# grossmanlev/FL-distributed-delay

Measured on AMD Instinct MI355X. Metric: simulated worker-steps/sec (node) @1024 workers, delay 50; aggregation HBM GB/s, higher is better.
Workload: dtype f32

## Files before the change

### fl-distributed-delay_amd/csrc/common.h

```cpp
#pragma once
#include <hip/hip_runtime.h>
#include <stdint.h>
#include <stdlib.h>

#define FLSIM_WAVE 64

#if !defined(FLSIM_LAB) &&                                                                  \
    (defined(FLSIM_X6_FRESH) || defined(FLSIM_X6_PP_V) || defined(FLSIM_DG_FMS) ||          \
     defined(FLSIM_DIRECT_FENCES) || defined(FLSIM_DX6_FENCES) || defined(FLSIM_BUFLOAD) ||  \
     defined(FLSIM_SEQ_EARLY_EXIT) || defined(FLSIM_X6_FLUSH) || defined(FLSIM_WGRAD_X6) ||     \
     defined(FLSIM_ZL1F) || defined(FLSIM_SINGLE_BUF) || defined(FLSIM_DG3_FM) || defined(FLSIM_DX_FM))
#error "FLSIM_* measurement overrides need a lab build (make LAB=1)"
#endif

typedef float f32x4 __attribute__((ext_vector_type(4)));

namespace flsim {

void set_error(const char* fmt, ...);
const char* last_error();

#define FLSIM_CHECK_HIP(expr)                                                           \
    do {                                                                                \
        hipError_t _e = (expr);                                                         \
        if (_e != hipSuccess) {                                                         \
            ::flsim::set_error("%s failed: %s (%s:%d)", #expr, hipGetErrorString(_e),   \
                               __FILE__, __LINE__);                                     \
            return 2;                                                                   \
        }                                                                               \
    } while (0)

#define FLSIM_REQUIRE(cond, ...)                                                        \
    do {                                                                                \
        if (!(cond)) {                                                                  \
            ::flsim::set_error(__VA_ARGS__);                                            \
            return 1;                                                                   \
        }                                                                               \
    } while (0)

#define RC(x) do { int _r = (x); if (_r) return _r; } while (0)

inline const char* lab_env(const char* name) {
#ifdef FLSIM_LAB
    return getenv(name);
// ... 54 lines not shown
```

### fl-distributed-delay_amd/csrc/gemm_direct.h

```cpp
#pragma once
#include "loaders.h"

namespace flsim {

#ifndef FLSIM_DIRECT_FENCES
#define FLSIM_DIRECT_FENCES 1
#endif
constexpr bool DIRECT_FENCES = FLSIM_DIRECT_FENCES;

template <int IH, int IW, int CI, int PAD, int FM, bool WIN = false, int OHX = 0,
          class SRC = BufSrc>
struct Im2colDirect {
    using Unit = typename SRC::Unit;
    static constexpr int PIX = SRC::SM ? GK : CI;
    static constexpr int SLICE = SRC::SM ? IH * IW * GK : GK;
    static constexpr int OH = OHX > 0 ? OHX : IH + 2 * PAD - 2;
    static constexpr int OW = OHX > 0 ? OHX : IW + 2 * PAD - 2;
    static constexpr int PH = OH / 2, PW = OW / 2;
    static constexpr int ROWS_PER_IMG = WIN ? 4 * PH * PW : OH * OW;
    static_assert(CI % 16 == 0, "direct A needs whole 16-channel slices");

    const float* X;
    const float* XL = nullptr;
    int M;
    unsigned vb[FM];
    unsigned short tapmask[FM];
    SRC buf;

    __device__ void setup(int r0, int lane) {
        const int q = lane >> 4;
        buf.init(X, XL, (unsigned long)((M + ROWS_PER_IMG - 1) / ROWS_PER_IMG) * IH * IW * CI * 4);
#pragma unroll
        for (int f = 0; f < FM; ++f) {
            const int m = r0 + 16 * f + (lane & 15);
            long base = 0;
            int msk = 0;
            if (m < M) {
                const int nimg = m / ROWS_PER_IMG;
                const int rem = m - nimg * ROWS_PER_IMG;
                int oh, ow;
                if constexpr (WIN) {
                    const int qq = rem >> 2;
                    const int ph = qq / PW;
                    oh = 2 * ph + ((rem >> 1) & 1);
                    ow = 2 * (qq - ph * PW) + (rem & 1);
                } else {
                    oh = rem / OW;
                    ow = rem - oh * OW;
                }
                base = (long)nimg * IH * IW * CI + ((long)(oh - PAD) * IW + (ow - PAD)) * PIX +
                       4 * q;
#pragma unroll
                for (int t = 0; t < 9; ++t) {
                    const int ih = oh + t / 3 - PAD, iw = ow + t % 3 - PAD;
                    if ((unsigned)ih < (unsigned)IH && (unsigned)iw < (unsigned)IW) msk |= 1 << t;
                }
            }
            vb[f] = (unsigned)base * 4u;
            tapmask[f] = (unsigned short)msk;
        }
    }
    __device__ void load(int ks, Unit (&r)[FM]) const {
        const int cs = ks / 9;
        const int khkw = ks - 9 * cs;
        const int kh = khkw / 3;
        const unsigned off = (unsigned)(((kh * IW + (khkw - 3 * kh)) * PIX + cs * SLICE) * 4);
#pragma unroll
        for (int f = 0; f < FM; ++f) r[f] = buf.ld_or0(vb[f] + off, (tapmask[f] >> khkw) & 1);
    }
};

template <int TR, int NT>
struct RowsKCStage {
    static constexpr int ROWS = TR;
    static constexpr bool KC = true;
    static constexpr int TOTAL = ROWS * 4;
    static constexpr int UNITS = (TOTAL + NT - 1) / NT;
    static constexpr int FLOATS = KCTile<ROWS>::FLOATS + 4;
    const float* P;
    long ld;
    int NR;
    unsigned rowb[UNITS];
    int dst[UNITS];
    BufSrc buf;
    __device__ void setup(int r0, int tid) {
        buf.init(P, (unsigned long)NR * ld * 4);
#pragma unroll
        for (int j = 0; j < UNITS; ++j) {
            const int u0 = tid + j * NT;
            const bool real = u0 < TOTAL;
            const int u = real ? u0 : u0 % TOTAL;
            const int r = u >> 2, q = u & 3;
            rowb[j] = r0 + r < NR ? (unsigned)(((long)(r0 + r) * ld + 4 * q) * 4) : BUF_OOB;
            dst[j] = real ? KCTile<ROWS>::chunk_off(r, q) : KCTile<ROWS>::FLOATS;
        }
    }
    __device__ void load(int ks, f32x4 (&r)[UNITS]) const {
#pragma unroll
        for (int j = 0; j < UNITS; ++j)
            r[j] = buf.ld(rowb[j] == BUF_OOB ? BUF_OOB : rowb[j] + (unsigned)(ks * GK * 4));
    }
    __device__ void store(float* lds, const f32x4 (&r)[UNITS]) const {
// ... 125 lines not shown
```

### fl-distributed-delay_amd/csrc/gemm_dx6.h

```cpp
#pragma once
#include "gemm_direct.h"
#include "gemm_x6.h"

namespace flsim {

#ifndef FLSIM_DX6_FENCES
#define FLSIM_DX6_FENCES 1
#endif
constexpr bool DX6_FENCES = FLSIM_DX6_FENCES;

template <int TR, int NT, int NPL>
struct RowsKCStageXs {
    using Unit = XsUnit;
    static constexpr int ROWS = TR;
    static constexpr bool KC = true;
    static constexpr int TOTAL = ROWS * 4;
    static constexpr int UNITS = (TOTAL + NT - 1) / NT;
    static constexpr int PLANE = KCTile<ROWS>::FLOATS;
    static constexpr int SPARE = NPL * PLANE;
    static constexpr int FLOATS = NPL * PLANE + 4;
    static_assert(NPL == 2 || NPL == 3, "");
    const float* P;
    const float* PL;
    long ld;
// ... 44 lines not shown
    constexpr int STAGE_LD = BN + 4;
    constexpr int BASE_FL = 2 * STG;
    constexpr int WROWS = 16 * FM;
    constexpr int WM_FIT = (BASE_FL > 8192 ? BASE_FL : 8192) / (WROWS * STAGE_LD);
    constexpr int WM_PASS = WM_FIT < 1 ? 1 : (WM_FIT > WAVES ? WAVES : WM_FIT);
    constexpr int LDS_FL = STAGED && WM_PASS * WROWS * STAGE_LD > BASE_FL
                               ? WM_PASS * WROWS * STAGE_LD : BASE_FL;
    static_assert(LDS_FL * 4 <= 160 * 1024, "LDS");
    __shared__ __attribute__((aligned(16))) float lds[LDS_FL];

    const int tid = threadIdx.x;
    const int lane = tid & 63;
    const int wave = tid >> 6;
    const int nb = gridDim.x;
    const int b = blockIdx.x;
    const int q = nb / 8, r = nb % 8, xcd = b % 8;
    const int L = (xcd < r ? xcd * (q + 1) : r * (q + 1) + (xcd - r) * q) + b / 8;
    const int tn = L % tiles_n;
    const int tm = L / tiles_n;
    const int m0 = tm * BM;
    const int n0 = tn * BN;

    ad.setup(m0 + wave * WROWS, lane);
    bl.setup(n0, tid);

    f32x4 acc[FM][FN];
#pragma unroll
    for (int i = 0; i < FM; ++i)
#pragma unroll
        for (int j = 0; j < FN; ++j) acc[i][j] = f32x4{0.f, 0.f, 0.f, 0.f};

    constexpr int R = DEPTH + 1;
    static_assert(KB % R == 0, "the A register ring index must be static");
    XsUnit ra[R][FM];
    typename BL::Unit rb[BL::UNITS];
    const int nst = ksteps / KB;
#pragma unroll
    for (int d = 0; d < DEPTH; ++d) ad.load(d, ra[d]);
#pragma unroll
    for (int kk = 0; kk < KB; ++kk) {
        bl.load(kk, rb);
        bl.store(lds + kk * BFL, rb);
    }
    __syncthreads();
    if constexpr (WAVES == 8) {
        if (wave >= 4) __builtin_amdgcn_s_setprio(1);
    }
    for (int s = 0; s < nst; ++s) {
        const float* Bs = lds + (s & 1) * STG;
        float* Bn = lds + ((s + 1) & 1) * STG;
        const int kn = (s + 1) * KB;
#pragma unroll
        for (int kk = 0; kk < KB; ++kk) {
            const int ks = s * KB + kk;
            if (kk > 0) bl.store(Bn + (kk - 1) * BFL, rb);
            bl.load(kn + kk, rb);
            ad.load(ks + DEPTH, ra[(kk + DEPTH) % R]);
            if constexpr (DX6_FENCES) __builtin_amdgcn_sched_barrier(0);
            const float* Bk = Bs + kk * BFL;
            f32x4 a0[FM], a1[FM];
#pragma unroll
            for (int i = 0; i < FM; ++i) {
                a0[i] = ra[kk % R][i].hm;
                a1[i] = xs_hl(ra[kk % R][i]);
            }
#pragma unroll
            for (int j = 0; j < FN; ++j) {
                const f32x4 x0 = read_frag<true, BN>(Bk, 16 * j, lane);
                const f32x4 x2 = read_frag<true, BN>(Bk + PLANE, 16 * j, lane);
                f32x4 x1;
                if constexpr (BFL >= 3 * PLANE)
                    x1 = read_frag<true, BN>(Bk + 2 * PLANE, 16 * j, lane);
                else
                    x1 = f32x4{x0.z, x0.w, x0.x, x0.y};
#pragma unroll
                for (int i = 0; i < FM; ++i) {
                    acc[i][j] = x6_step<x6_fresh(true)>(acc[i][j], a0[i], a1[i], x0, x1, x2);
                }
            }
            if constexpr (DX6_FENCES) __builtin_amdgcn_sched_barrier(0);
        }
        bl.store(Bn + (KB - 1) * BFL, rb);
        __syncthreads();
    }

    if constexpr (STAGED) {
        static_assert(BN == EPI::NCOL || (IsPartial<EPI>::value && EPI::NCOL % BN == 0),
                      "staged epilogue needs the full row in one block");
        constexpr int PASSES = (WAVES + WM_PASS - 1) / WM_PASS;
#pragma unroll 1
        for (int pass = 0; pass < PASSES; ++pass) {
            __syncthreads();
            if (wave / WM_PASS == pass) {
#pragma unroll
                for (int i = 0; i < FM; ++i)
#pragma unroll
                    for (int j = 0; j < FN; ++j) {
                        const int ml = (wave - pass * WM_PASS) * WROWS + 16 * i + 4 * (lane >> 4);
                        const int nl = 16 * j + (lane & 15);
#pragma unroll
                        for (int rr = 0; rr < 4; ++rr)
                            lds[(ml + rr) * STAGE_LD + nl] = epi.value(nl, acc[i][j][rr]);
                    }
            }
            __syncthreads();
            const int w_hi = (pass + 1) * WM_PASS < WAVES ? (pass + 1) * WM_PASS : WAVES;
            staged_store(epi, lds, STAGE_LD, m0 + pass * WM_PASS * WROWS,
                         (w_hi - pass * WM_PASS) * WROWS, n0, BN, tid, 64 * WAVES);
        }
    } else {
#pragma unroll
        for (int i = 0; i < FM; ++i)
#pragma unroll
            for (int j = 0; j < FN; ++j) {
                const int m = m0 + wave * WROWS + 16 * i + 4 * (lane >> 4);
                const int n = n0 + 16 * j + (lane & 15);
// ... 7 lines not shown
```

### fl-distributed-delay_amd/csrc/net_kernels.h

```cpp
#pragma once
#include "epi_xs.h"
#include "gemm_direct.h"
#include "gemm_dx6.h"
#include "gemm_x6.h"
#include "loaders.h"
#include "pn1.h"
#include "probe.h"

namespace flsim {

static __global__ void __launch_bounds__(256)
k_fill_batch(const uint8_t* __restrict__ pool, const int32_t* __restrict__ labels,
             const int32_t* __restrict__ list_a, int len_a, const int32_t* __restrict__ list_b,
             int len_b, const WorkerRec* __restrict__ workers, int n_workers_total, uint64_t seed,
             const float* __restrict__ lut, float* __restrict__ x0, int32_t* __restrict__ y) {
    const int s = blockIdx.x;
    const int w = s / SAMPLES_PER_WORKER;
    const int j = s - w * SAMPLES_PER_WORKER;
    const WorkerRec wr = workers[w];
    const uint32_t bsz = wr.pad ? wr.pad : (uint32_t)SAMPLES_PER_WORKER;
    const uint32_t q = (wr.i >> 20) * SAMPLES_PER_WORKER + (uint32_t)j;
    float* out = x0 + (long)s * 4096;
    if (q >= bsz) {
        if (threadIdx.x == 0) y[s] = -1;
// ... 810 lines not shown
    al.NC = CO;
    BL bl;
    bl.X = X;
    bl.M = M;
    EpiSlabAccRing epi{{slab, CO, KP, (long)CO * KP, bslab, zinit}};
    const int tm = ceil_div(CO, BM), tn = KP / BN;
    static const int cap =
        resident_blocks((const void*)gemm_kernel<FM, FN, WM, WN, AL, BL, EpiSlabAccRing>, NT);
    const int ksteps = ceil_div(M, GK);
    const int zu = wsplit(ksteps, Z, tm * tn, cap);
    if (zused) *zused = zu;
    const int per = (ksteps + zu - 1) / zu;
    const ProbeSlot ps = probe_begin();
    hipExtLaunchKernelGGL((gemm_kernel<FM, FN, WM, WN, AL, BL, EpiSlabAccRing>), dim3(tm * tn * zu),
                          dim3(NT), 0, st, ps.start, ps.stop, 0, al, bl, epi, ksteps, per, tm, tn);
    FLSIM_LAUNCH_CHECK();
    return probe_end(ps, kid, 2.0 * M * CO * kreal);
}

template <int IH, int IW, int CI, int PAD, int FM, int FN, int WM, int WN, int FMS, int FNS,
          int WMS, int WNS, int VO = 0, bool DZC = false, bool X6 = false, class SRC = BufSrc,
          class SRCB = SRC>
static int conv_wgrad_sz(const float* dz, const float* X, int S, int CO, int KP, float* slab,
                         float* bslab, int Z, hipStream_t st, int kid, int kreal, int zinit,
                         int* zused, const float* dzl = nullptr, const float* Xl = nullptr) {
    if (S <= small_chunk_samples())
        return conv_wgrad<IH, IW, CI, PAD, FMS, FNS, WMS, WNS, VO, DZC, X6, SRC, SRCB>(
            dz, X, S, CO, KP, slab, bslab, Z, st, kid, kreal, zinit, zused, dzl, Xl);
    return conv_wgrad<IH, IW, CI, PAD, FM, FN, WM, WN, VO, DZC, X6, SRC, SRCB>(
        dz, X, S, CO, KP, slab, bslab, Z, st, kid, kreal, zinit, zused, dzl, Xl);
}

template <int IH, int IW, int CI, int PAD, int FM, int FN, int WAVES, int KB, int DEPTH, int NPL,
          bool WIN, int OHX, class ASRC = XsSrc, class EPI>
static int conv_dx6(XsT X, int S, XsT W, int N, int KP, const EPI& epi, hipStream_t st, int kid,
                    int kreal) {
    static_assert(ASRC::SPLIT, "split input");
    using AD = Im2colDirect<IH, IW, CI, PAD, FM, WIN, OHX, ASRC>;
    using BL = RowsKCStageXs<16 * FN, 64 * WAVES, NPL>;
    constexpr int BM = 16 * FM * WAVES, BN = 16 * FN;
    FLSIM_REQUIRE((KP / GK) % KB == 0, "direct GEMM: %d k-steps not a multiple of %d", KP / GK, KB);
    AD ad;
    ad.X = X.hm;
    ad.XL = X.l;
    ad.M = S * AD::ROWS_PER_IMG;
    BL bl;
    bl.P = W.hm;
    bl.PL = W.l;
    bl.ld = KP;
    bl.NR = N;
    const int tm = ceil_div(ad.M, BM), tn = ceil_div(N, BN);
    const ProbeSlot ps = probe_begin();
    hipExtLaunchKernelGGL((gemm_dx6_kernel<FM, FN, WAVES, KB, DEPTH, AD, BL, EPI>),
                          dim3(tm * tn), dim3(64 * WAVES), 0, st, ps.start, ps.stop, 0, ad, bl,
                          epi, KP / GK, tm, tn);
    FLSIM_LAUNCH_CHECK();
    return probe_end(ps, kid, 2.0 * ad.M * N * kreal);
}

template <int IH, int IW, int CI, int PAD, int FM, int FN, int WM, int WN, bool WIN, int OHX,
          class EPI>
static int conv_xs(XsT X, int S, XsT W, int N, int KP, const EPI& epi, hipStream_t st, int kid,
                   int kreal) {
    constexpr int NT = 64 * WM * WN;
    constexpr int BM = 16 * FM * WM, BN = 16 * FN * WN;
    using AL = Im2colKC<IH, IW, CI, PAD, BM, NT, WIN, OHX, XsSrc>;
    using BL = RowsKC<BN, NT, XsSrc>;
    AL al;
    al.X = X.hm;
    al.XL = X.l;
    al.M = S * AL::ROWS_PER_IMG;
// ... 77 lines not shown
```

### fl-distributed-delay_amd/csrc/pn1_net.hip

```cpp
#include <stdarg.h>
#include <stdio.h>
#include <string.h>

#include <mutex>
#include <unordered_map>

#include "net_kernels.h"
#include "slabstep.h"

namespace flsim {

static thread_local char g_err[512];
void set_error(const char* fmt, ...) {
    va_list ap;
    va_start(ap, fmt);
    vsnprintf(g_err, sizeof(g_err), fmt, ap);
    va_end(ap);
}
const char* last_error() { return g_err; }

struct ConvGeo {
    int CI, CIP, CO, H;
    int KP;
    int ZW;
// ... 214 lines not shown
#pragma unroll
                for (int r = 0; r < 4; ++r)
                    st[(16 * t + 4 * g + r) * C1_LD + 16 * j + i] = fmaxf(acc[t][j][r] + bj[j], 0.f);
        __builtin_amdgcn_wave_barrier();
#pragma unroll
        for (int q0 = 0; q0 < C1_ROWS * 12; q0 += 64) {
            const int q = q0 + lane, slice = q >> 7, row = (q & 127) >> 2, c4 = 4 * slice + (q & 3);
            xs_store_f(a1, a1l, a1f, xs_unit<48, 1156, true>((unsigned)(u * C1_ROWS + row), c4),
                       *reinterpret_cast<const f32x4*>(st + row * C1_LD + 4 * c4));
        }
        __builtin_amdgcn_wave_barrier();
    }
}

static int conv1_fwd(const float* x0, const float* W, const float* bias, XsT a1, float* a1f,
                     int S, hipStream_t st) {
    const long M = (long)S * 34 * 34;
    if (M % C1_ROWS) return 1;
    const long units = M / C1_ROWS;
    const int grid = (int)(units / 4 < 2048 ? (units + 3) / 4 : 2048);
    const ProbeSlot ps = probe_begin();
    hipExtLaunchKernelGGL(k_conv1_fwd, dim3(grid), dim3(256), 0, st, ps.start, ps.stop, 0, x0, W,
                          bias, a1.hm, a1.l, a1f, units);
    FLSIM_LAUNCH_CHECK();
    return probe_end(ps, K_FWD1, 2.0 * M * 48 * 27);
}

#ifndef FLSIM_DX_FM
#define FLSIM_DX_FM 4
#endif
constexpr int DX_FM = FLSIM_DX_FM, DX_FMS = 1, DX_KB = 3, DX_DEPTH = 2, DX_NPL = 2;


template <int IH, int IW, int CI, int PAD, int FN, bool WIN, int OHX, int FM = DX_FM,
          int WAVES = 8, int FMS = (FM == DX_FM ? DX_FMS : FM / 2), class EPI>
static int dx6(XsT X, int S, XsT W, int N, int KP, const EPI& epi, hipStream_t st, int kid,
               int kreal) {
    if (S <= small_chunk_samples())
        return conv_dx6<IH, IW, CI, PAD, FMS, FN, WAVES, DX_KB, DX_DEPTH, DX_NPL, WIN, OHX,
                        XsSrcSM>(X, S, W, N, KP, epi, st, kid, kreal);
    return conv_dx6<IH, IW, CI, PAD, FM, FN, WAVES, DX_KB, DX_DEPTH, DX_NPL, WIN, OHX, XsSrcSM>(
        X, S, W, N, KP, epi, st, kid, kreal);
}

template <int IH, int IW, int CI, int PAD, int FM, int FN, int WM, int WN, bool WIN, int OHX,
          class EPI>
static int xs(XsT X, int S, XsT W, int N, int KP, const EPI& epi, hipStream_t st, int kid,
              int kreal) {
    if (S <= small_chunk_samples())
        return conv_xs<IH, IW, CI, PAD, FM / 2, FN, WM, WN, WIN, OHX>(X, S, W, N, KP, epi, st, kid,
                                                                     kreal);
    return conv_xs<IH, IW, CI, PAD, FM, FN, WM, WN, WIN, OHX>(X, S, W, N, KP, epi, st, kid, kreal);
}

static int forward(const GradState& g, const WS& w, const float* theta, int S,
                   const WorkerRec* workers, uint64_t seed, int dropout, hipStream_t st) {
    const XsT a1 = w.x(w.a1, w.a1l), d1 = w.x(w.d1, w.d1l), a3 = w.x(w.a3, w.a3l);
    const XsT d2 = w.x(w.d2, w.d2l), a5 = w.x(w.a5, w.a5l);
    RC(conv1_fwd(w.x0, theta + P_OFF[0], theta + P_OFF[1], a1, w.a1f, S, st));
    RC((dx6<34, 34, 48, 2, 3, true, 0, 4, 4, 2>(a1, S, g.wfx[1], 48, 432,
        EpiPoolDropXs<18, 18, 48, true>{d1.hm, d1.l, w.i1, theta + P_OFF[3], workers, seed, SITE_DROP1,
                                  THR_P25, SCALE_P25, dropout, S * 18 * 18 * 4, w.d1f}, st,
        K_FWD2, 432)));
    RC((dx6<18, 18, 48, 2, 6, false, 0>(d1, S, g.wfx[2], 96, 432,
        EpiBiasReluXs<96, true, 400>{a3.hm, a3.l, theta + P_OFF[5], S * 20 * 20, w.a3f}, st, K_FWD3,
        432)));
    RC((dx6<20, 20, 96, 2, 6, true, 0>(a3, S, g.wfx[3], 96, 864,
        EpiPoolDropXs<11, 11, 96>{d2.hm, d2.l, w.i2, theta + P_OFF[7], workers, seed, SITE_DROP2,
                                  THR_P25, SCALE_P25, dropout, S * 11 * 11 * 4, w.d2f}, st,
        K_FWD4, 864)));
    RC((xs<11, 11, 96, 2, 4, 6, 4, 2, false, 0>(d2, S, g.wfx[4], 192, 864,
        EpiBiasReluXs<192>{a5.hm, a5.l, theta + P_OFF[9], S * 13 * 13, w.a5f}, st, K_FWD5, 864)));
    RC((xs<13, 13, 192, 2, 4, 6, 4, 2, true, 0>(a5, S, g.wfx[5], 192, 1728,
        EpiPoolDrop<7, 7, 192, true>{w.d3, w.i3, theta + P_OFF[11], workers, seed, SITE_DROP3,
                                     THR_P25, SCALE_P25, dropout, S * 7 * 7 * 4}, st, K_FWD6,
        1728)));
    if (S <= 2048)
        RC((linear_fwd<1, 2, 2, 2, true, EpiSlabStoreFresh>(w.d3, theta + P_OFF[12], w.part, S,
                                                            512, 9408, ZL1F, st, K_L1F)));
    else if (S <= 4096)
        RC((linear_fwd<2, 2, 2, 2, true, EpiSlabStoreFresh>(w.d3, theta + P_OFF[12], w.part, S,
                                                            512, 9408, ZL1F, st, K_L1F)));
    else
        RC((linear_fwd<4, 4, 2, 2, true, EpiSlabStoreFresh>(w.d3, theta + P_OFF[12], w.part, S,
                                                            512, 9408, ZL1F, st, K_L1F)));
    RC(linear_finish(w.part, ZL1F, theta + P_OFF[13], w.e1, S, 512, workers, seed, SITE_DROP4,
                     THR_P50, SCALE_P50, dropout, st));
    RC((linear_fwd<2, 2, 2, 2>(w.e1, theta + P_OFF[14], w.part, S, 256, 512, 1, st, K_L2F)));
    RC(linear_finish(w.part, 1, theta + P_OFF[15], w.e2, S, 256, workers, seed, SITE_DROP5,
                     THR_P50, SCALE_P50, dropout, st));
    return 0;
}

struct EpochRows {
    int z[8];
};
static std::mutex g_rows_mu;
static std::unordered_map<const void*, EpochRows> g_rows;

static EpochRows* epoch_rows(const void* gradstate) {
// ... 269 lines not shown

long flsim_pn1_gradstate_bytes(void) { return gs_layout(nullptr).total_floats * 4; }

long flsim_pn1_workspace_bytes(int max_samples) { return ws_layout(nullptr, max_samples).bytes; }

int flsim_pn1_workspace_offset(int which, int samples, long* offset_bytes) {
    char* const fake = reinterpret_cast<char*>(4096);
    WS w = ws_layout(fake, samples);
    const void* p[] = {w.x0, w.a1, w.a2, w.d1, w.a3, w.a4, w.d2, w.a5, w.a6, w.d3,
                       w.e1, w.e2, w.dh1, w.dh2, w.gx, w.gy, w.loss_s, w.dlog, w.y,
                       w.i1, w.i2, w.i3,
                       w.a1l, w.d1l, w.a3l, w.d2l, w.a5l, w.a6l, w.a4l, w.a2l, w.gxl,
                       w.a1f, w.d1f, w.a3f, w.d2f, w.a5f};
    FLSIM_REQUIRE(which >= 0 && which < (int)(sizeof(p) / sizeof(p[0])), "bad workspace id %d", which);
    *offset_bytes = (long)((const char*)p[which] - fake);
    return 0;
}

int flsim_pn1_workspace_split_part(int which) {
    switch (which) {
        case 1: return 22;
        case 3: return 23;
        case 4: return 24;
        case 6: return 25;
        case 7: return 26;
        default: return -1;
    }
}

int flsim_pn1_workspace_slice_major(int which) {
    return which == 1 || which == 3 || which == 4;
}

int flsim_pn1_begin_epoch(void* gradstate, const float* theta, hipStream_t stream) {
    FLSIM_REQUIRE(gradstate && theta, "null pointer");
    RC(pipe_join(gradstate, stream));
    GradState g = gs_layout((float*)gradstate);
    RC(pack_weights(g, theta, stream));
    FLSIM_CHECK_HIP(hipMemsetAsync(g.l3w, 0, (g.l3b + ZH * 10 - g.l3w) * 4, stream));
    FLSIM_CHECK_HIP(hipMemsetAsync((float*)gradstate + g.cnt_off, 0,
                                   step_counter_floats(g.plan) * 4, stream));
    std::lock_guard<std::mutex> lk(g_rows_mu);
    g_rows[gradstate] = EpochRows{{0, 0, 0, 0, 0, 0, 0, 0}};
    return 0;
}

void flsim_pn1_release(void* gradstate) {
    pipe_release(gradstate);
    std::lock_guard<std::mutex> lk(g_rows_mu);
    g_rows.erase(gradstate);
}

static int run_chunk(void* gradstate, const WS& w, const float* theta, const WorkerRec* workers,
                     int n_chunk_workers, uint64_t seed, int dropout, int backward_pass,
                     float* worker_loss, hipStream_t stream,
                     float gscale = 1.f / SAMPLES_PER_WORKER) {
    const int S = n_chunk_workers * SAMPLES_PER_WORKER;
    GradState g = gs_layout((float*)gradstate);
    RC(forward(g, w, theta, S, workers, seed, dropout, stream));
    RC(head_and_loss<256>(w.e2, theta + P_OFF[16], theta + P_OFF[17], w.y, w.loss_s, w.dlog, w.dh2,
                          S, backward_pass, dropout ? SCALE_P50 : 1.f, gscale, worker_loss,
                          stream, workers));
    if (backward_pass) {
        EpochRows* er = epoch_rows(gradstate);
        FLSIM_REQUIRE(er, "backward pass without flsim_pn1_begin_epoch on this gradstate");
        RC(backward(g, w, theta, S, dropout, stream, er));
// ... 315 lines not shown
```

### fl-distributed-delay_amd/flsim/_lib.py

```python
from __future__ import annotations

import ctypes
import os

import torch

LIB_PATH = os.environ.get("FLSIM_LIB") or os.path.join(os.path.dirname(os.path.abspath(__file__)),
                                                        "_lib", "libflsim.so")

EXPORTS = [
    "flsim_last_error", "flsim_sched_create", "flsim_sched_destroy", "flsim_sched_epoch",
    "flsim_sched_state", "flsim_pn1_param_count", "flsim_pn1_gradstate_bytes",
    "flsim_pn1_workspace_bytes", "flsim_pn1_workspace_offset", "flsim_pn1_workspace_split_part",
    "flsim_pn1_workspace_slice_major", "flsim_pn1_begin_epoch",
    "flsim_pn1_fwd_bwd_chunk", "flsim_pn1_fwd_bwd_input", "flsim_pn1_end_epoch",
    "flsim_pn1_eval_pool", "flsim_vgg11_param_count", "flsim_vgg11_gradstate_bytes",
    "flsim_vgg11_workspace_bytes", "flsim_vgg11_workspace_offset", "flsim_vgg11_begin_epoch",
    "flsim_vgg11_fwd_bwd_chunk", "flsim_vgg11_fwd_bwd_input", "flsim_vgg11_end_epoch",
    "flsim_vgg11_eval_pool", "flsim_vgg11_bn_param_count", "flsim_vgg11_bn_gradstate_bytes",
    "flsim_vgg11_bn_workspace_bytes", "flsim_vgg11_bn_workspace_offset",
    "flsim_vgg11_bn_stats_per_worker", "flsim_vgg11_bn_begin_epoch",
    "flsim_vgg11_bn_fwd_bwd_chunk", "flsim_vgg11_bn_fwd_bwd_input", "flsim_vgg11_bn_end_epoch",
    "flsim_vgg11_bn_eval_pool", "flsim_vgg11_bn_update_running",
    "flsim_pn1_eval_input", "flsim_vgg11_eval_input", "flsim_vgg11_bn_eval_input",
    "flsim_pn1_server_step", "flsim_vgg11_server_step", "flsim_vgg11_bn_server_step",
    "flsim_aggregate_adam", "flsim_aggregate_adam_rule", "flsim_aggregate_adam_sum",
    "flsim_cascade_program", "flsim_cascade_eval_host",
    "flsim_probe_enable", "flsim_probe_read", "flsim_probe_disable",
    "flsim_probe_kernel_count", "flsim_probe_kernel_name", "flsim_pn1_release",
    "flsim_pn1_fwd_bwd_chunk_async", "flsim_pn1_fwd_bwd_input_async",
    "flsim_aggregate_adam_rule_push", "flsim_pn1_fwd_rows", "flsim_pn1_bwd_rows",
    "flsim_pn1_load_rows", "flsim_pn1_fwd_loaded_rows", "flsim_vgg11_load_rows",
    "flsim_vgg11_fwd_bwd_loaded_rows", "flsim_vgg11_bn_load_rows",
    "flsim_vgg11_bn_fwd_bwd_loaded_rows",
    "flsim_comm_unique_id", "flsim_comm_create", "flsim_comm_size", "flsim_comm_rank",
    "flsim_allreduce_sum", "flsim_comm_destroy",
    "flsim_aggregate_optim_rule_push", "flsim_pn1_server_step_optim",
    "flsim_vgg11_server_step_optim", "flsim_vgg11_bn_server_step_optim",
]
COMM_ID_BYTES = 128


class FLSimError(RuntimeError):
    pass


MAX_ARRAYS = 64


class FlsimRule(ctypes.Structure):
    _fields_ = [("k", ctypes.c_int32), ("c", ctypes.c_int32), ("prog", ctypes.c_void_p),
                ("info", ctypes.c_int32 * 4), ("n_arrays", ctypes.c_int32),
                ("arrays", ctypes.c_void_p * MAX_ARRAYS)]


OPT_KINDS = {"adam": 0, "adamw": 1, "sgd": 2}


class FlsimOptim(ctypes.Structure):
    _fields_ = [("kind", ctypes.c_int32), ("nesterov", ctypes.c_int32), ("lr", ctypes.c_double),
                ("beta1", ctypes.c_double), ("beta2", ctypes.c_double), ("eps", ctypes.c_double),
                ("weight_decay", ctypes.c_double), ("momentum", ctypes.c_double),
                ("dampening", ctypes.c_double)]


class WorkerRec(ctypes.Structure):
    _fields_ = [("t", ctypes.c_uint32), ("i", ctypes.c_uint32), ("k", ctypes.c_uint32),
                ("pad", ctypes.c_uint32)]


_L = None
# ... 75 lines not shown
    L.flsim_aggregate_adam_sum.argtypes = [
        vp, ctypes.c_int, vp, vp, vp, ctypes.c_long, vp, ctypes.c_int,
        ctypes.c_long, ctypes.c_double, ctypes.c_double, ctypes.c_double, ctypes.c_double, vp]
    L.flsim_aggregate_adam_rule.argtypes = [
        vp, vp, vp, vp, vp, ctypes.c_long, vp, ctypes.c_int,
        ctypes.c_long, ctypes.c_double, ctypes.c_double, ctypes.c_double, ctypes.c_double, vp]
    L.flsim_aggregate_adam_rule_push.argtypes = [
        vp, vp, vp, vp, vp, vp, ctypes.c_long, vp, ctypes.c_int,
        ctypes.c_long, ctypes.c_double, ctypes.c_double, ctypes.c_double, ctypes.c_double, vp]
    L.flsim_aggregate_optim_rule_push.argtypes = [
        vp, vp, vp, vp, vp, vp, ctypes.c_long, vp, ctypes.c_int, ctypes.c_long, vp, vp]
    L.flsim_cascade_program.argtypes = [ctypes.c_int, vp, vp, ctypes.c_int, vp, ctypes.c_int, vp]
    L.flsim_cascade_eval_host.argtypes = [vp, vp, vp, vp, ctypes.c_int, vp, ctypes.c_long, vp]
    L.flsim_probe_enable.argtypes = [ctypes.c_int]
    L.flsim_probe_read.argtypes = [vp, vp, vp]
    L.flsim_probe_kernel_name.restype = ctypes.c_char_p
    L.flsim_probe_kernel_name.argtypes = [ctypes.c_int]
    _L = L
    return L


def check(rc):
    if rc != 0:
        msg = lib().flsim_last_error().decode(errors="replace")
        if rc == 1:
            if "IndexError" in msg:
                raise IndexError(msg)
            if "ZeroDivisionError" in msg:
                raise ZeroDivisionError(msg)
            raise ValueError(msg)
        raise FLSimError(msg)


def ptr(t):
    return ctypes.c_void_p(t.data_ptr()) if t is not None else ctypes.c_void_p(0)


def stream_ptr(device=None):
    return ctypes.c_void_p(torch.cuda.current_stream(device).cuda_stream)


class KernelProbe:

    def __init__(self, capacity=20000):
        check(lib().flsim_probe_enable(capacity))

    def read(self):
        import numpy as np
        n = lib().flsim_probe_kernel_count()
        cnt = np.zeros(n, np.int32)
        ms = np.zeros(n, np.float64)
        fl = np.zeros(n, np.float64)
        check(lib().flsim_probe_read(cnt.ctypes.data_as(vp), ms.ctypes.data_as(vp),
                                     fl.ctypes.data_as(vp)))
        return {lib().flsim_probe_kernel_name(k).decode(): (int(cnt[k]), float(ms[k]), float(fl[k]))
                for k in range(n) if cnt[k]}

    def close(self):
        check(lib().flsim_probe_disable())
```

### include/flsim.h

```cpp
#ifndef FLSIM_H
#define FLSIM_H

#include <stddef.h>
#include <stdint.h>

#ifdef __cplusplus
extern "C" {
#endif

typedef struct ihipStream_t* flsim_stream_t;

typedef struct WorkerRec {
    uint32_t t;
    uint32_t i;
    uint32_t k;
    uint32_t pad;
} WorkerRec;

const char* flsim_last_error(void);

#define FLSIM_COMM_ID_BYTES 128
typedef struct flsim_comm flsim_comm;
int flsim_comm_unique_id(unsigned char* id );
int flsim_comm_create(int nranks, int rank, const unsigned char* id, flsim_comm** out);
int flsim_comm_size(const flsim_comm* comm);
int flsim_comm_rank(const flsim_comm* comm);
int flsim_allreduce_sum(flsim_comm* comm, float* buf, size_t count, flsim_stream_t stream);
int flsim_comm_destroy(flsim_comm* comm);

#define FLSIM_DELAY_ZERO ((int32_t)0x80000000)
typedef struct flsim_sched flsim_sched;
flsim_sched* flsim_sched_create(int32_t n, const int32_t* delays, int32_t throttle,
                                int32_t max_throttle);
void flsim_sched_destroy(flsim_sched* s);
int flsim_sched_epoch(flsim_sched* s, uint8_t* computes, uint8_t* fast, int32_t* stale_worker,
                      int64_t* stale_src, int64_t* info);
void flsim_sched_state(const flsim_sched* s, int64_t* out3);

long flsim_pn1_param_count(void);
long flsim_pn1_gradstate_bytes(void);
long flsim_pn1_workspace_bytes(int max_samples);
int flsim_pn1_workspace_offset(int which, int samples, long* offset_bytes);
int flsim_pn1_workspace_split_part(int which);
int flsim_pn1_workspace_slice_major(int which);
int flsim_pn1_begin_epoch(void* gradstate, const float* theta, flsim_stream_t stream);
int flsim_pn1_fwd_bwd_chunk(void* gradstate, void* workspace, int max_samples, const float* theta,
                            const uint8_t* pool, const int32_t* labels, const int32_t* list_a,
                            int len_a, const int32_t* list_b, int len_b, const float* lut,
                            const WorkerRec* workers, int n_chunk_workers, int n_workers_total,
                            uint64_t seed, int dropout, int backward_pass, float* worker_loss,
                            flsim_stream_t stream);
int flsim_pn1_fwd_bwd_chunk_async(void* gradstate, void* workspace, int max_samples,
                                  const float* theta, const uint8_t* pool, const int32_t* labels,
                                  const int32_t* list_a, int len_a, const int32_t* list_b,
                                  int len_b, const float* lut, const WorkerRec* workers,
                                  int n_chunk_workers, int n_workers_total, uint64_t seed,
                                  int dropout, float* worker_loss, flsim_stream_t stream);
int flsim_pn1_fwd_bwd_input_async(void* gradstate, void* workspace, int max_samples,
                                  const float* theta, const float* x, const int64_t* y,
                                  int n_samples, const WorkerRec* workers, uint64_t seed,
                                  int dropout, float* worker_loss, flsim_stream_t stream);
int flsim_pn1_fwd_rows(void* gradstate, void* workspace, int max_samples, int row0,
                       const float* theta, const float* x, const int64_t* y, int n_samples,
                       const WorkerRec* workers, uint64_t seed, int dropout, float* worker_loss,
                       flsim_stream_t stream);
int flsim_pn1_load_rows(void* gradstate, void* workspace, int max_samples, int row0,
                        const float* x, const int64_t* y, int n_samples, flsim_stream_t stream);
int flsim_pn1_fwd_loaded_rows(void* gradstate, void* workspace, int max_samples, int row0,
                              int n_rows, const float* theta, const WorkerRec* workers,
                              uint64_t seed, int dropout, float* worker_loss,
                              flsim_stream_t stream);
int flsim_pn1_bwd_rows(void* gradstate, void* workspace, int max_samples, int n_rows,
                       const float* theta, int dropout, flsim_stream_t stream);
int flsim_pn1_fwd_bwd_input(void* gradstate, void* workspace, int max_samples, const float* theta,
                            const float* x, const int64_t* y, int n_samples,
                            const WorkerRec* workers, uint64_t seed, int dropout,
                            int backward_pass, float* worker_loss, flsim_stream_t stream);
// ... 150 lines not shown
```

Before: 1164.

## Derive middle 3x3 conv tap from neighbour lanes via DPP instead of loading

```diff
diff --git a/fl-distributed-delay_amd/csrc/common.h b/fl-distributed-delay_amd/csrc/common.h
--- a/fl-distributed-delay_amd/csrc/common.h
+++ b/fl-distributed-delay_amd/csrc/common.h
@@ -9,7 +9,8 @@
     (defined(FLSIM_X6_FRESH) || defined(FLSIM_X6_PP_V) || defined(FLSIM_DG_FMS) ||          \
      defined(FLSIM_DIRECT_FENCES) || defined(FLSIM_DX6_FENCES) || defined(FLSIM_BUFLOAD) ||  \
      defined(FLSIM_SEQ_EARLY_EXIT) || defined(FLSIM_X6_FLUSH) || defined(FLSIM_WGRAD_X6) ||     \
-     defined(FLSIM_ZL1F) || defined(FLSIM_SINGLE_BUF) || defined(FLSIM_DG3_FM) || defined(FLSIM_DX_FM))
+     defined(FLSIM_ZL1F) || defined(FLSIM_SINGLE_BUF) || defined(FLSIM_DG3_FM) || defined(FLSIM_DX_FM) || \
+     defined(FLSIM_MIDTAP2) || defined(FLSIM_MIDTAP3) || defined(FLSIM_MIDTAP4))
 #error "FLSIM_* measurement overrides need a lab build (make LAB=1)"
 #endif
 
diff --git a/fl-distributed-delay_amd/csrc/gemm_direct.h b/fl-distributed-delay_amd/csrc/gemm_direct.h
--- a/fl-distributed-delay_amd/csrc/gemm_direct.h
+++ b/fl-distributed-delay_amd/csrc/gemm_direct.h
@@ -8,9 +8,81 @@
 #endif
 constexpr bool DIRECT_FENCES = FLSIM_DIRECT_FENCES;
 
+struct MidTapSrc {
+    int lane;
+    int kw;
+};
+__host__ __device__ constexpr MidTapSrc midtap_src(bool win, int lane) {
+    if (win) return MidTapSrc{lane ^ 1, (lane & 1) ? 2 : 0};
+    return (lane & 15) < 15 ? MidTapSrc{lane + 1, 0} : MidTapSrc{lane - 1, 2};
+}
+
+constexpr int DPP_QUAD_SWAP = 0xB1;
+constexpr int DPP_ROW_SHL1 = 0x101;
+constexpr int DPP_ROW_SHR1 = 0x111;
+constexpr int dpp_src_lane(int ctrl, int lane) {
+    return ctrl == DPP_QUAD_SWAP  ? (lane ^ 1)
+         : ctrl == DPP_ROW_SHL1   ? ((lane & 15) < 15 ? lane + 1 : -1)
+         : ctrl == DPP_ROW_SHR1   ? ((lane & 15) > 0 ? lane - 1 : -1)
+                                  : -2;
+}
+constexpr bool midtap_dpp_matches(bool win) {
+    for (int l = 0; l < 64; ++l) {
+        const MidTapSrc s = midtap_src(win, l);
+        if (win) {
+            if (dpp_src_lane(DPP_QUAD_SWAP, l) != s.lane) return false;
+            if (midtap_src(true, s.lane).kw == s.kw) return false;
+        } else {
+            const int from0 = dpp_src_lane(DPP_ROW_SHL1, l), from2 = dpp_src_lane(DPP_ROW_SHR1, l);
+            if (s.kw == 0 ? from0 != s.lane : (from0 != -1 || from2 != s.lane)) return false;
+        }
+    }
+    return true;
+}
+static_assert(midtap_dpp_matches(false) && midtap_dpp_matches(true), "DPP controls vs midtap_src");
+
+template <bool WIN>
+__device__ __forceinline__ int midtap_dword(int k0, int k2, bool send2) {
+    if constexpr (WIN) {
+        const int s = send2 ? k2 : k0;
+        return __builtin_amdgcn_update_dpp(s, s, DPP_QUAD_SWAP, 0xf, 0xf, true);
+    } else {
+        const int hi = __builtin_amdgcn_update_dpp(k2, k2, DPP_ROW_SHR1, 0xf, 0xf, true);
+        return __builtin_amdgcn_update_dpp(hi, k0, DPP_ROW_SHL1, 0xf, 0xf, false);
+    }
+}
+typedef int i32x4 __attribute__((ext_vector_type(4)));
+typedef int i32x2 __attribute__((ext_vector_type(2)));
+template <bool WIN>
+__device__ __forceinline__ f32x4 midtap_unit(f32x4 k0, f32x4 k2, bool send2) {
+    const i32x4 a = __builtin_bit_cast(i32x4, k0), b = __builtin_bit_cast(i32x4, k2);
+    i32x4 r;
+#pragma unroll
+    for (int e = 0; e < 4; ++e) r[e] = midtap_dword<WIN>(a[e], b[e], send2);
+    return __builtin_bit_cast(f32x4, r);
+}
+template <bool WIN>
+__device__ __forceinline__ f32x2 midtap_unit(f32x2 k0, f32x2 k2, bool send2) {
+    const i32x2 a = __builtin_bit_cast(i32x2, k0), b = __builtin_bit_cast(i32x2, k2);
+    i32x2 r;
+#pragma unroll
+    for (int e = 0; e < 2; ++e) r[e] = midtap_dword<WIN>(a[e], b[e], send2);
+    return __builtin_bit_cast(f32x2, r);
+}
+template <bool WIN>
+__device__ __forceinline__ XsUnit midtap_unit(const XsUnit& k0, const XsUnit& k2, bool send2) {
+    return XsUnit{midtap_unit<WIN>(k0.hm, k2.hm, send2), midtap_unit<WIN>(k0.l, k2.l, send2)};
+}
+
 template <int IH, int IW, int CI, int PAD, int FM, bool WIN = false, int OHX = 0,
-          class SRC = BufSrc>
+          class SRC = BufSrc, int MID = 0>
 struct Im2colDirect {
+    static constexpr bool MIDTAP = MID != 0;
+    static constexpr bool MIDTAP_TWOROW = MID == 2;
+    static_assert(MID >= 0 && MID <= 2, "");
+    static_assert(!MID || (PAD == 2 && OHX == 0),
+                  "the middle tap is a neighbour's outer tap only when OW = IW + 2: with padding "
+                  "0 or 1 (or a cropped output) the identity fails at the row ends");
     using Unit = typename SRC::Unit;
     static constexpr int PIX = SRC::SM ? GK : CI;
     static constexpr int SLICE = SRC::SM ? IH * IW * GK : GK;
@@ -68,6 +140,13 @@
 #pragma unroll
         for (int f = 0; f < FM; ++f) r[f] = buf.ld_or0(vb[f] + off, (tapmask[f] >> khkw) & 1);
     }
+    __device__ void midtap(const Unit (&k0)[FM], const Unit (&k2)[FM], Unit (&k1)[FM],
+                           int lane) const {
+        static_assert(MID, "");
+        const bool send2 = midtap_src(WIN, lane).kw == 0;
+#pragma unroll
+        for (int f = 0; f < FM; ++f) k1[f] = midtap_unit<WIN>(k0[f], k2[f], send2);
+    }
 };
 
 template <int TR, int NT>
diff --git a/fl-distributed-delay_amd/csrc/gemm_dx6.h b/fl-distributed-delay_amd/csrc/gemm_dx6.h
--- a/fl-distributed-delay_amd/csrc/gemm_dx6.h
+++ b/fl-distributed-delay_amd/csrc/gemm_dx6.h
@@ -100,11 +100,18 @@
 
     constexpr int R = DEPTH + 1;
     static_assert(KB % R == 0, "the A register ring index must be static");
+    constexpr bool MID = AD::MIDTAP;
+    static_assert(!MID || (KB == 3 && DEPTH == 2), "MIDTAP: a stage is one filter row");
     XsUnit ra[R][FM];
     typename BL::Unit rb[BL::UNITS];
     const int nst = ksteps / KB;
-#pragma unroll
-    for (int d = 0; d < DEPTH; ++d) ad.load(d, ra[d]);
+    if constexpr (MID) {
+        ad.load(0, ra[0]);
+        ad.load(2, ra[2]);
+    } else {
+#pragma unroll
+        for (int d = 0; d < DEPTH; ++d) ad.load(d, ra[d]);
+    }
 #pragma unroll
     for (int kk = 0; kk < KB; ++kk) {
         bl.load(kk, rb);
@@ -114,42 +121,100 @@
     if constexpr (WAVES == 8) {
         if (wave >= 4) __builtin_amdgcn_s_setprio(1);
     }
-    for (int s = 0; s < nst; ++s) {
-        const float* Bs = lds + (s & 1) * STG;
-        float* Bn = lds + ((s + 1) & 1) * STG;
-        const int kn = (s + 1) * KB;
-#pragma unroll
-        for (int kk = 0; kk < KB; ++kk) {
-            const int ks = s * KB + kk;
-            if (kk > 0) bl.store(Bn + (kk - 1) * BFL, rb);
-            bl.load(kn + kk, rb);
-            ad.load(ks + DEPTH, ra[(kk + DEPTH) % R]);
-            if constexpr (DX6_FENCES) __builtin_amdgcn_sched_barrier(0);
-            const float* Bk = Bs + kk * BFL;
-            f32x4 a0[FM], a1[FM];
+    auto mma = [&](const float* Bk, const XsUnit (&u)[FM]) {
+        if constexpr (DX6_FENCES) __builtin_amdgcn_sched_barrier(0);
+        f32x4 a0[FM], a1[FM];
+#pragma unroll
+        for (int i = 0; i < FM; ++i) {
+            a0[i] = u[i].hm;
+            a1[i] = xs_hl(u[i]);
+        }
+#pragma unroll
+        for (int j = 0; j < FN; ++j) {
+            const f32x4 x0 = read_frag<true, BN>(Bk, 16 * j, lane);
+            const f32x4 x2 = read_frag<true, BN>(Bk + PLANE, 16 * j, lane);
+            f32x4 x1;
+            if constexpr (BFL >= 3 * PLANE)
+                x1 = read_frag<true, BN>(Bk + 2 * PLANE, 16 * j, lane);
+            else
+                x1 = f32x4{x0.z, x0.w, x0.x, x0.y};
 #pragma unroll
             for (int i = 0; i < FM; ++i) {
-                a0[i] = ra[kk % R][i].hm;
-                a1[i] = xs_hl(ra[kk % R][i]);
-            }
-#pragma unroll
-            for (int j = 0; j < FN; ++j) {
-                const f32x4 x0 = read_frag<true, BN>(Bk, 16 * j, lane);
-                const f32x4 x2 = read_frag<true, BN>(Bk + PLANE, 16 * j, lane);
-                f32x4 x1;
-                if constexpr (BFL >= 3 * PLANE)
-                    x1 = read_frag<true, BN>(Bk + 2 * PLANE, 16 * j, lane);
-                else
-                    x1 = f32x4{x0.z, x0.w, x0.x, x0.y};
+                acc[i][j] = x6_step<x6_fresh(true)>(acc[i][j], a0[i], a1[i], x0, x1, x2);
+            }
+        }
+        if constexpr (DX6_FENCES) __builtin_amdgcn_sched_barrier(0);
+    };
+    if constexpr (!MID) {
+        for (int s = 0; s < nst; ++s) {
+            const float* Bs = lds + (s & 1) * STG;
+            float* Bn = lds + ((s + 1) & 1) * STG;
+            const int kn = (s + 1) * KB;
+#pragma unroll
+            for (int kk = 0; kk < KB; ++kk) {
+                const int ks = s * KB + kk;
+                if (kk > 0) bl.store(Bn + (kk - 1) * BFL, rb);
+                bl.load(kn + kk, rb);
+                ad.load(ks + DEPTH, ra[(kk + DEPTH) % R]);
+                if constexpr (DX6_FENCES) __builtin_amdgcn_sched_barrier(0);
+                const float* Bk = Bs + kk * BFL;
+                f32x4 a0[FM], a1[FM];
 #pragma unroll
                 for (int i = 0; i < FM; ++i) {
-                    acc[i][j] = x6_step<x6_fresh(true)>(acc[i][j], a0[i], a1[i], x0, x1, x2);
+                    a0[i] = ra[kk % R][i].hm;
+                    a1[i] = xs_hl(ra[kk % R][i]);
                 }
-            }
-            if constexpr (DX6_FENCES) __builtin_amdgcn_sched_barrier(0);
-        }
-        bl.store(Bn + (KB - 1) * BFL, rb);
-        __syncthreads();
+#pragma unroll
+                for (int j = 0; j < FN; ++j) {
+                    const f32x4 x0 = read_frag<true, BN>(Bk, 16 * j, lane);
+                    const f32x4 x2 = read_frag<true, BN>(Bk + PLANE, 16 * j, lane);
+                    f32x4 x1;
+                    if constexpr (BFL >= 3 * PLANE)
+                        x1 = read_frag<true, BN>(Bk + 2 * PLANE, 16 * j, lane);
+                    else
+                        x1 = f32x4{x0.z, x0.w, x0.x, x0.y};
+#pragma unroll
+                    for (int i = 0; i < FM; ++i) {
+                        acc[i][j] = x6_step<x6_fresh(true)>(acc[i][j], a0[i], a1[i], x0, x1, x2);
+                    }
+                }
+                if constexpr (DX6_FENCES) __builtin_amdgcn_sched_barrier(0);
+            }
+            bl.store(Bn + (KB - 1) * BFL, rb);
+            __syncthreads();
+        }
+    } else {
+        constexpr bool TWOROW = AD::MIDTAP_TWOROW;
+        auto row = [&](int s, auto odd) {
+            constexpr int U2 = TWOROW && decltype(odd)::value ? 1 : 2;
+            constexpr int N2 = TWOROW ? 3 - U2 : 2;
+            const float* Bs = lds + (s & 1) * STG;
+            float* Bn = lds + ((s + 1) & 1) * STG;
+            const int kn = (s + 1) * KB;
+            bl.load(kn, rb);
+            mma(Bs, ra[0]);
+            bl.store(Bn, rb);
+            bl.load(kn + 1, rb);
+            XsUnit mid[FM];
+            ad.midtap(ra[0], ra[U2], mid, lane);
+            ad.load(kn, ra[0]);
+            mma(Bs + BFL, mid);
+            bl.store(Bn + BFL, rb);
+            bl.load(kn + 2, rb);
+            if constexpr (TWOROW) ad.load(kn + 2, ra[N2]);
+            mma(Bs + 2 * BFL, ra[U2]);
+            if constexpr (!TWOROW) ad.load(kn + 2, ra[N2]);
+            bl.store(Bn + 2 * BFL, rb);
+            __syncthreads();
+        };
+        int s = 0;
+        if constexpr (TWOROW) {
+            for (; s + 1 < nst; s += 2) {
+                row(s, std::false_type{});
+                row(s + 1, std::true_type{});
+            }
+        }
+        for (; s < nst; ++s) row(s, std::false_type{});
     }
 
     if constexpr (STAGED) {
diff --git a/fl-distributed-delay_amd/csrc/net_kernels.h b/fl-distributed-delay_amd/csrc/net_kernels.h
--- a/fl-distributed-delay_amd/csrc/net_kernels.h
+++ b/fl-distributed-delay_amd/csrc/net_kernels.h
@@ -866,11 +866,11 @@
 }
 
 template <int IH, int IW, int CI, int PAD, int FM, int FN, int WAVES, int KB, int DEPTH, int NPL,
-          bool WIN, int OHX, class ASRC = XsSrc, class EPI>
+          bool WIN, int OHX, class ASRC = XsSrc, int MID = 0, class EPI>
 static int conv_dx6(XsT X, int S, XsT W, int N, int KP, const EPI& epi, hipStream_t st, int kid,
                     int kreal) {
     static_assert(ASRC::SPLIT, "split input");
-    using AD = Im2colDirect<IH, IW, CI, PAD, FM, WIN, OHX, ASRC>;
+    using AD = Im2colDirect<IH, IW, CI, PAD, FM, WIN, OHX, ASRC, MID>;
     using BL = RowsKCStageXs<16 * FN, 64 * WAVES, NPL>;
     constexpr int BM = 16 * FM * WAVES, BN = 16 * FN;
     FLSIM_REQUIRE((KP / GK) % KB == 0, "direct GEMM: %d k-steps not a multiple of %d", KP / GK, KB);
diff --git a/fl-distributed-delay_amd/csrc/pn1_net.hip b/fl-distributed-delay_amd/csrc/pn1_net.hip
--- a/fl-distributed-delay_amd/csrc/pn1_net.hip
+++ b/fl-distributed-delay_amd/csrc/pn1_net.hip
@@ -270,15 +270,25 @@
 constexpr int DX_FM = FLSIM_DX_FM, DX_FMS = 1, DX_KB = 3, DX_DEPTH = 2, DX_NPL = 2;
 
 
-template <int IH, int IW, int CI, int PAD, int FN, bool WIN, int OHX, int FM = DX_FM,
+#ifndef FLSIM_MIDTAP2
+#define FLSIM_MIDTAP2 2
+#endif
+#ifndef FLSIM_MIDTAP3
+#define FLSIM_MIDTAP3 1
+#endif
+#ifndef FLSIM_MIDTAP4
+#define FLSIM_MIDTAP4 1
+#endif
+
+template <int IH, int IW, int CI, int PAD, int FN, bool WIN, int OHX, int MID, int FM = DX_FM,
           int WAVES = 8, int FMS = (FM == DX_FM ? DX_FMS : FM / 2), class EPI>
 static int dx6(XsT X, int S, XsT W, int N, int KP, const EPI& epi, hipStream_t st, int kid,
                int kreal) {
     if (S <= small_chunk_samples())
         return conv_dx6<IH, IW, CI, PAD, FMS, FN, WAVES, DX_KB, DX_DEPTH, DX_NPL, WIN, OHX,
-                        XsSrcSM>(X, S, W, N, KP, epi, st, kid, kreal);
-    return conv_dx6<IH, IW, CI, PAD, FM, FN, WAVES, DX_KB, DX_DEPTH, DX_NPL, WIN, OHX, XsSrcSM>(
-        X, S, W, N, KP, epi, st, kid, kreal);
+                        XsSrcSM, MID>(X, S, W, N, KP, epi, st, kid, kreal);
+    return conv_dx6<IH, IW, CI, PAD, FM, FN, WAVES, DX_KB, DX_DEPTH, DX_NPL, WIN, OHX, XsSrcSM,
+                    MID>(X, S, W, N, KP, epi, st, kid, kreal);
 }
 
 template <int IH, int IW, int CI, int PAD, int FM, int FN, int WM, int WN, bool WIN, int OHX,
@@ -296,14 +306,14 @@
     const XsT a1 = w.x(w.a1, w.a1l), d1 = w.x(w.d1, w.d1l), a3 = w.x(w.a3, w.a3l);
     const XsT d2 = w.x(w.d2, w.d2l), a5 = w.x(w.a5, w.a5l);
     RC(conv1_fwd(w.x0, theta + P_OFF[0], theta + P_OFF[1], a1, w.a1f, S, st));
-    RC((dx6<34, 34, 48, 2, 3, true, 0, 4, 4, 2>(a1, S, g.wfx[1], 48, 432,
+    RC((dx6<34, 34, 48, 2, 3, true, 0, FLSIM_MIDTAP2, 4, 4, 2>(a1, S, g.wfx[1], 48, 432,
         EpiPoolDropXs<18, 18, 48, true>{d1.hm, d1.l, w.i1, theta + P_OFF[3], workers, seed, SITE_DROP1,
                                   THR_P25, SCALE_P25, dropout, S * 18 * 18 * 4, w.d1f}, st,
         K_FWD2, 432)));
-    RC((dx6<18, 18, 48, 2, 6, false, 0>(d1, S, g.wfx[2], 96, 432,
+    RC((dx6<18, 18, 48, 2, 6, false, 0, FLSIM_MIDTAP3>(d1, S, g.wfx[2], 96, 432,
         EpiBiasReluXs<96, true, 400>{a3.hm, a3.l, theta + P_OFF[5], S * 20 * 20, w.a3f}, st, K_FWD3,
         432)));
-    RC((dx6<20, 20, 96, 2, 6, true, 0>(a3, S, g.wfx[3], 96, 864,
+    RC((dx6<20, 20, 96, 2, 6, true, 0, FLSIM_MIDTAP4>(a3, S, g.wfx[3], 96, 864,
         EpiPoolDropXs<11, 11, 96>{d2.hm, d2.l, w.i2, theta + P_OFF[7], workers, seed, SITE_DROP2,
                                   THR_P25, SCALE_P25, dropout, S * 11 * 11 * 4, w.d2f}, st,
         K_FWD4, 864)));
@@ -639,6 +649,15 @@
     return which == 1 || which == 3 || which == 4;
 }
 
+int flsim_midtap_lane(int win, int lane, int* src_lane, int* src_kw) {
+    FLSIM_REQUIRE(src_lane && src_kw, "null pointer");
+    FLSIM_REQUIRE(lane >= 0 && lane < FLSIM_WAVE, "lane %d outside the wave", lane);
+    const MidTapSrc s = midtap_src(win != 0, lane);
+    *src_lane = s.lane;
+    *src_kw = s.kw;
+    return 0;
+}
+
 int flsim_pn1_begin_epoch(void* gradstate, const float* theta, hipStream_t stream) {
     FLSIM_REQUIRE(gradstate && theta, "null pointer");
     RC(pipe_join(gradstate, stream));
diff --git a/fl-distributed-delay_amd/flsim/_lib.py b/fl-distributed-delay_amd/flsim/_lib.py
--- a/fl-distributed-delay_amd/flsim/_lib.py
+++ b/fl-distributed-delay_amd/flsim/_lib.py
@@ -37,6 +37,7 @@
     "flsim_allreduce_sum", "flsim_comm_destroy",
     "flsim_aggregate_optim_rule_push", "flsim_pn1_server_step_optim",
     "flsim_vgg11_server_step_optim", "flsim_vgg11_bn_server_step_optim",
+    "flsim_midtap_lane",
 ]
 COMM_ID_BYTES = 128
 
@@ -178,6 +179,14 @@
         raise FLSimError(msg)
 
 
+def midtap_lane(win, lane):
+    fn = lib().flsim_midtap_lane
+    fn.argtypes = [ctypes.c_int, ctypes.c_int, vp, vp]
+    src, kw = ctypes.c_int(), ctypes.c_int()
+    check(fn(int(bool(win)), int(lane), ctypes.byref(src), ctypes.byref(kw)))
+    return src.value, kw.value
+
+
 def ptr(t):
     return ctypes.c_void_p(t.data_ptr()) if t is not None else ctypes.c_void_p(0)
 
diff --git a/include/flsim.h b/include/flsim.h
--- a/include/flsim.h
+++ b/include/flsim.h
@@ -43,6 +43,7 @@
 int flsim_pn1_workspace_offset(int which, int samples, long* offset_bytes);
 int flsim_pn1_workspace_split_part(int which);
 int flsim_pn1_workspace_slice_major(int which);
+int flsim_midtap_lane(int win, int lane, int* src_lane, int* src_kw);
 int flsim_pn1_begin_epoch(void* gradstate, const float* theta, flsim_stream_t stream);
 int flsim_pn1_fwd_bwd_chunk(void* gradstate, void* workspace, int max_samples, const float* theta,
                             const uint8_t* pool, const int32_t* labels, const int32_t* list_a,
```

After: 1171, median of 6. About the same (+0.6%).
